# DiWu9/Union-Thesis-SLAM

Hardware: AMD Instinct MI355X
Metric: depth frames/sec (640x480 into 512^3 @ 2 cm dense TSDF; hash alongside) (higher is better)
Workload: dtype f64

## Files before the change

### union-thesis-slam_amd/csrc/tsdf_dense.hip

```cpp
#include <algorithm>
#include <vector>
#include <cstdlib>
#include <cstring>

#include "tsdf_host.h"

using namespace tsdf;

struct tsdf_dense {
    Base b;
    Mesh mesh;
    int nz = 4;
    bool fused = true;
    int gi_per_cu = 0;
};

namespace {

__global__ void k_fill3(float* t, float* w, float* c, size_t n) {
    for (size_t i = (size_t)blockIdx.x * blockDim.x + threadIdx.x; i < n;
         i += (size_t)gridDim.x * blockDim.x) {
        t[i] = 1.0f;
        w[i] = 0.0f;
        c[i] = 0.0f;
// ... 460 lines not shown
        if (e == hipSuccess) e = hipMalloc(&uc, hb);
        if (e == hipSuccess) e = hipMemcpyAsync(ut, halo_tsdf, hb, hipMemcpyHostToDevice, B.stream);
        if (e == hipSuccess) e = hipMemcpyAsync(uc, halo_color, hb, hipMemcpyHostToDevice, B.stream);
        if (e != hipSuccess) r = set_error(TSDF_E_HIP, "halo upload: %s", hipGetErrorString(e));
        ht = ut;
        hc = uc;
    } else if (n_halo > 0) {
        TSDF_HIP(hipDeviceSynchronize());
    }
    if (r == TSDF_OK) r = extract_mesh(B, B.pool, h->mesh, d, ht, hc);
    if (ut) (void)hipFree(ut);
    if (uc) (void)hipFree(uc);
    TSDF_TRY(r);
    *n_verts = h->mesh.n_verts;
    *n_tris = h->mesh.n_tris;
    return TSDF_OK;
}

int tsdf_dense_get_mesh(tsdf_dense_t* h, float* verts, float* normals, uint8_t* colors, int32_t* faces) {
    if (!h) return set_error(TSDF_E_ARG, "null handle");
    TSDF_HIP(hipSetDevice(h->b.device));
    return copy_mesh(h->b, h->mesh, verts, normals, colors, faces);
}

int tsdf_dense_get_mesh_keys(tsdf_dense_t* h, int64_t* keys) {
    if (!h || !keys) return set_error(TSDF_E_ARG, "null pointer");
    TSDF_HIP(hipSetDevice(h->b.device));
    return copy_mesh(h->b, h->mesh, nullptr, nullptr, nullptr, nullptr, keys);
}

int tsdf_dense_get_rows(tsdf_dense_t* h, const int64_t* rows, int64_t n_rows, float* tsdf_, float* weight_,
                        float* color_, int flags) {
    if (!h || n_rows < 0 || (n_rows > 0 && !rows)) return set_error(TSDF_E_ARG, "bad arguments");
    Base& B = h->b;
    TSDF_HIP(hipSetDevice(B.device));
    TSDF_TRY(dense_flush(h));
    if (n_rows == 0) return TSDF_OK;
    for (int64_t i = 0; i < n_rows; ++i)
        if (rows[i] < 0 || rows[i] >= B.vol.dims[0])
            return set_error(TSDF_E_ARG, "local row %lld outside [0, %d)", (long long)rows[i], B.vol.dims[0]);
    const size_t yz = (size_t)B.vol.dims[1] * B.vol.dims[2];
    const size_t bytes = (size_t)n_rows * yz * sizeof(float);
    DevPtrs bufs;
    long long* drows = nullptr;
    TSDF_HIP(hipMalloc(&drows, sizeof(long long) * n_rows));
    bufs.p.push_back(drows);
    TSDF_HIP(hipMemcpyAsync(drows, rows, sizeof(long long) * n_rows, hipMemcpyHostToDevice, B.stream));
    float* out[3] = {tsdf_, weight_, color_};
    float* dev[3] = {B.pool.tsdf, B.pool.weight, B.pool.color};
    const unsigned grid = (unsigned)std::min<size_t>(((size_t)n_rows * yz + 255) / 256, (size_t)B.n_cu * 16);
    for (int k = 0; k < 3; ++k) {
        if (!out[k]) continue;
        float* dst = out[k];
        if (!(flags & TSDF_DEVICE_PTRS)) {
            TSDF_HIP(hipMalloc(&dst, bytes));
            bufs.p.push_back(dst);
        }
        hipLaunchKernelGGL(k_rows<true>, dim3(grid), dim3(256), 0, B.stream, B.vol, (const long long*)drows, 0ll,
                           (long long)n_rows, dev[k], dst);
        TSDF_HIP(hipGetLastError());
        if (!(flags & TSDF_DEVICE_PTRS)) TSDF_HIP(hipMemcpyAsync(out[k], dst, bytes, hipMemcpyDeviceToHost, B.stream));
    }
    TSDF_HIP(hipStreamSynchronize(B.stream));
    return TSDF_OK;
}

int tsdf_dense_set_profiling(tsdf_dense_t* h, int on) {
    if (!h) return set_error(TSDF_E_ARG, "null handle");
    TSDF_HIP(hipSetDevice(h->b.device));
    TSDF_TRY(dense_flush(h));
    return h->b.set_profiling(on);
}

}

#ifdef TSDF_WG_TIMES
extern "C" int tsdf_diag_wg_times(unsigned long long* out) {
    TSDF_HIP(hipDeviceSynchronize());
    TSDF_HIP(hipMemcpyFromSymbol(out, HIP_SYMBOL(g_wg_times), sizeof(unsigned long long) * 4 * kWgTimes));
    static const std::vector<unsigned long long> zero(4 * (size_t)kWgTimes, 0ull);
    TSDF_HIP(hipMemcpyToSymbol(HIP_SYMBOL(g_wg_times), zero.data(), sizeof(unsigned long long) * 4 * kWgTimes));
    return TSDF_OK;
}
#endif

#ifdef TSDF_DIAG
extern "C" int tsdf_diag_counts(unsigned long long* out) {
    TSDF_HIP(hipDeviceSynchronize());
    TSDF_HIP(hipMemcpyFromSymbol(out, HIP_SYMBOL(tsdf::g_ddiag), sizeof(unsigned long long) * 8));
    const unsigned long long zero[8] = {};
    TSDF_HIP(hipMemcpyToSymbol(HIP_SYMBOL(tsdf::g_ddiag), zero, sizeof(zero)));
    return TSDF_OK;
}
#endif
```

### union-thesis-slam_amd/csrc/tsdf_device.h

```cpp
#pragma once
#include <hip/hip_runtime.h>
#include <stdint.h>
#include <type_traits>

namespace tsdf {

constexpr int kBrickEdge = 8;
constexpr int kBrickVox = 512;
constexpr int kWG = 256;
constexpr int kPyrLevels = 6;
constexpr int kStatSpread = 64;
constexpr unsigned long long kEmpty = ~0ull;
constexpr unsigned long long kTomb = ~0ull - 1ull;

enum Stat { ST_VOXELS = 0, ST_VISITED, ST_TOUCHED, ST_ALLOC, ST_PROBE, ST_LOOKUPS, ST_OVERFLOW,
            ST_PROBE_MAX, ST_BAD_ENTRY, ST_UNIQUE, kNStat };

struct Vol {
    int dims[3];
    int off[3];
    int xstride;
    int xodd;
    int sb[3];
    int nb[3];
// ... 97 lines not shown
    long long tombs;
    long long seq;
};

struct Table {
    unsigned long long* keys;
    int* vals;
    unsigned long long* occ;
    int* free_list;
    ListEntry* overflow;
    PoolState* st;
    PoolReport* rb;
    long long capacity;
    long long shard_cap;
    long long max_blocks;
    const int* owned;
    int n_owned;
    int* ins_list;
    long long ins_cap;
    int overflow_cap;
    int int_bits;
};

template <bool POW2 = false>
__host__ __device__ inline long long ref_hash(long long x, long long y, long long z, long long n,
                                              int int_bits) {
    const unsigned long long P1 = 73856093ull, P2 = 19349669ull, P3 = 83492791ull;
    long long h;
    if (int_bits == 32) {
        const int a = (int)(unsigned)((unsigned long long)x * P1);
        const int b = (int)(unsigned)((unsigned long long)y * P2);
        const int c = (int)(unsigned)((unsigned long long)z * P3);
        h = (long long)(a ^ b ^ c);
    } else {
        h = (long long)(((unsigned long long)x * P1) ^ ((unsigned long long)y * P2) ^
                        ((unsigned long long)z * P3));
    }
    if (POW2 || (n & (n - 1)) == 0) return h & (n - 1);
    long long m = h % n;
    return m < 0 ? m + n : m;
}

template <bool POW2 = false>
__host__ __device__ inline int shard_of(long long home, int n_shards, long long cap) {
    if (POW2 || (cap & (cap - 1)) == 0) return (int)((home * n_shards) >> (63 - __builtin_clzll((unsigned long long)cap)));
    return (int)((home * n_shards) / cap);
}

__host__ __device__ inline unsigned long long pack_key(int bx, int by, int bz) {
    return (unsigned long long)bx | ((unsigned long long)by << 21) | ((unsigned long long)bz << 42);
}

__device__ inline int lane_id() { return threadIdx.x & 63; }

__device__ unsigned long long fcmp64_mask(double a, double b, int pred) __asm("llvm.amdgcn.fcmp.i64.f64");
__device__ unsigned long long fcmp32_mask(float a, float b, int pred) __asm("llvm.amdgcn.fcmp.i64.f32");
__device__ unsigned long long icmp32_mask(unsigned a, unsigned b, int pred) __asm("llvm.amdgcn.icmp.i64.i32");
constexpr int kCmpOGT = 2, kCmpOGE = 3, kCmpOLT = 4, kCmpUNE = 14, kCmpNE = 33, kCmpULT = 36, kCmpSGT = 38;
__device__ inline bool lane_in(unsigned long long m) { return __builtin_amdgcn_inverse_ballot_w64(m); }
__device__ inline void sel_in_place(float& x, float y, unsigned long long m) {
    asm("v_cndmask_b32 %0, %0, %1, %2" : "+v"(x) : "v"(y), "s"(m));
}

template <typename T>
__device__ inline T coh_load(T* p) {
    return __hip_atomic_load(p, __ATOMIC_RELAXED, __HIP_MEMORY_SCOPE_AGENT);
}
template <typename T>
__device__ inline void coh_store(T* p, T v) {
    __hip_atomic_store(p, v, __ATOMIC_RELAXED, __HIP_MEMORY_SCOPE_AGENT);
}

__device__ inline double vox_world(float origin, double vs, int g) {
    return (double)(float)((double)origin + vs * (double)g);
}

struct BrickBox {
    double p0[3];
    float ext[3];
    float ctr[3];
    float rad;
};

__device__ inline BrickBox brick_box(const Vol& v, const double* eye, int bx, int by, int bz, int nx = 1,
                                     int ny = 1, int nz = 1) {
    const int bb[3] = {bx, by, bz}, nn[3] = {nx, ny, nz};
    BrickBox r;
#pragma unroll
    for (int a = 0; a < 3; ++a) {
        const int lo = bb[a] * kBrickEdge;
        const int hi = min(lo + nn[a] * kBrickEdge - 1, v.dims[a] - 1);
        const int glo = (a == 0) ? col_gx(v, bb[0]) : lo;
        const int ghi = (a == 0) ? col_gx(v, hi >> 3) + (hi & 7) : hi;
        r.p0[a] = (double)v.origin[a] + v.vs * (double)(glo + v.off[a]);
        r.ext[a] = (float)(v.vs * (double)(ghi - glo));
        r.ctr[a] = (float)(r.p0[a] + 0.5 * v.vs * (double)(ghi - glo) - eye[a]);
    }
    r.rad = 0.5f * sqrtf(r.ext[0] * r.ext[0] + r.ext[1] * r.ext[1] + r.ext[2] * r.ext[2]) + 1e-4f;
    return r;
}

__device__ inline bool cull_brick(const Vol& v, const Frame& fr, const PyrGeo& pg, const BrickBox& bb) {
#pragma unroll
    for (int i = 0; i < 5; ++i) {
        const float* q = fr.planes[i];
        if (q[0] * bb.ctr[0] + q[1] * bb.ctr[1] + q[2] * bb.ctr[2] + q[3] < -bb.rad) return false;
    }
    const double* T = fr.T;
    float c0[3], d[3][3];
#pragma unroll
    for (int r = 0; r < 3; ++r) {
        c0[r] = (float)(T[4 * r + 0] * bb.p0[0] + T[4 * r + 1] * bb.p0[1] + T[4 * r + 2] * bb.p0[2] + T[4 * r + 3]);
#pragma unroll
        for (int a = 0; a < 3; ++a) d[r][a] = (float)T[4 * r + a] * bb.ext[a];
    }
    const float fx = (float)fr.fx, fy = (float)fr.fy, cx = (float)fr.cx, cy = (float)fr.cy;
    float zmin = 3e38f, zmax = -3e38f, umin = 3e38f, umax = -3e38f, vmin = 3e38f, vmax = -3e38f;
#pragma unroll
    for (int c = 0; c < 8; ++c) {
        float q[3];
#pragma unroll
        for (int r = 0; r < 3; ++r)
            q[r] = c0[r] + ((c & 1) ? d[r][0] : 0.0f) + ((c & 2) ? d[r][1] : 0.0f) + ((c & 4) ? d[r][2] : 0.0f);
        zmin = fminf(zmin, q[2]);
        zmax = fmaxf(zmax, q[2]);
        const float iz = __builtin_amdgcn_rcpf(fmaxf(q[2], 1e-6f));
        const float u = fx * q[0] * iz + cx, w = fy * q[1] * iz + cy;
        umin = fminf(umin, u); umax = fmaxf(umax, u);
        vmin = fminf(vmin, w); vmax = fmaxf(vmax, w);
    }
    if (zmax < -1e-4f) return false;
    int u0 = 0, u1 = fr.W - 1, v0 = 0, v1 = fr.H - 1;
    if (zmin > 0.2f) {
        const float fu0 = floorf(umin) - 1.0f, fu1 = ceilf(umax) + 1.0f;
        const float fv0 = floorf(vmin) - 1.0f, fv1 = ceilf(vmax) + 1.0f;
        if (fu1 < 0.0f || fv1 < 0.0f || fu0 > (float)(fr.W - 1) || fv0 > (float)(fr.H - 1)) return false;
        u0 = (int)fmaxf(fu0, 0.0f); u1 = (int)fminf(fu1, (float)(fr.W - 1));
        v0 = (int)fmaxf(fv0, 0.0f); v1 = (int)fminf(fv1, (float)(fr.H - 1));
    }
    int L = 1;
    while (L < kPyrLevels && (((u1 >> L) - (u0 >> L)) > 3 || ((v1 >> L) - (v0 >> L)) > 3)) ++L;
    const float need = zmin - (float)v.trunc - 1e-3f;
    const int tx0 = u0 >> L, tx1 = u1 >> L, ty0 = v0 >> L, ty1 = v1 >> L;
    if (tx1 - tx0 > 3 || ty1 - ty0 > 3) return true;
    const float* lvl = fr.pyr + pg.off[L];
    const int wl = pg.w[L];
    float dmax = 0.0f;
#pragma unroll
    for (int dy = 0; dy < 4; ++dy)
#pragma unroll
        for (int dx = 0; dx < 4; ++dx)
            if (ty0 + dy <= ty1 && tx0 + dx <= tx1) dmax = fmaxf(dmax, lvl[(ty0 + dy) * wl + tx0 + dx]);
    return dmax > 0.0f && dmax >= need;
}

__device__ inline int pool_alloc(const Table& t) {
    const long long c = (long long)atomicAdd((unsigned long long*)&t.st->cursor, 1ull);
    const long long nf = coh_load(&t.st->free_count);
    const long long b = (c < nf) ? (long long)coh_load(&t.free_list[nf - 1 - c])
                                 : coh_load(&t.st->pool_top) + (c - nf);
    return (b < t.max_blocks) ? (int)b : -2;
}

__device__ inline int table_find_or_insert(const Table& t, unsigned long long key, long long home,
                                           bool insert, bool& is_new, long long& slot_out,
                                           long long& probe) {
    const int lane = lane_id();
    is_new = false;
    long long pos = home;
    long long tomb = -1;
    int blk = -1;
    for (long long scanned = 0; scanned < t.capacity + 64;) {
        long long s = pos + lane;
        if (s >= t.capacity) s -= t.capacity;
        if (s >= t.capacity) s %= t.capacity;
        const unsigned long long kk = coh_load(&t.keys[s]);
        const int vv = coh_load(&t.vals[s]);
        const unsigned long long hit = __ballot(kk == key);
        if (hit) {
            const int l = __ffsll((long long)hit) - 1;
            slot_out = __shfl(s, l);
            probe = scanned + l;
            return __shfl(vv, l);
        }
        const unsigned long long emp = __ballot(kk == kEmpty);
        unsigned long long tm = __ballot(kk == kTomb);
        if (emp) tm &= (emp & (~emp + 1)) - 1;
        if (tomb < 0 && tm) tomb = __shfl(s, __ffsll((long long)tm) - 1);
        if (emp) {
            if (!insert) return -1;
            const int le = __ffsll((long long)emp) - 1;
            const long long target = tomb >= 0 ? tomb : __shfl(s, le);
            const unsigned long long expect = tomb >= 0 ? kTomb : kEmpty;
            int ok = 0;
            if (lane == 0) {
                if (blk < 0) blk = pool_alloc(t);
                if (blk >= 0) {
                    const unsigned long long old = atomicCAS(&t.keys[target], expect, key);
                    if (old == expect) {
                        coh_store(&t.vals[target], blk);
                        ok = 1;
                    } else if (old == key) {
                        ok = 2;
                    }
                }
            }
            blk = __shfl(blk, 0);
            ok = __shfl(ok, 0);
            if (blk == -2) return -1;
            if (ok == 1) {
                is_new = true;
                slot_out = target;
                probe = scanned + ((target - pos + t.capacity) % t.capacity);
                return blk;
            }
            if (ok == 2) {
                slot_out = target;
                probe = scanned + ((target - pos + t.capacity) % t.capacity);
                return coh_load(&t.vals[target]);
            }
            scanned += (target - pos + t.capacity) % t.capacity + 1;
            pos = target + 1;
            if (pos >= t.capacity) pos -= t.capacity;
            tomb = -1;
            continue;
        }
        pos += 64;
        if (pos >= t.capacity) pos -= t.capacity;
        scanned += 64;
    }
    return -1;
}


__device__ unsigned short buf_ld_u16(__amdgpu_buffer_rsrc_t r, int vindex, int voffset, int soffset,
                                     int aux) __asm("llvm.amdgcn.struct.ptr.buffer.load.i16");
// ... 651 lines not shown
__device__ inline void append_kept(const Vol& v, ListEntry* list, unsigned int* count, unsigned long long* s_stat,
                                   int* res, unsigned e, unsigned fmask, int ncls, const Table* tab = nullptr,
                                   const Pool* pool = nullptr) {
    const int lane = lane_id();
    const int cls = __popc(fmask);
    const unsigned long long any = __ballot(cls != 0);
    if (!any) return;
    unsigned n_cls = 0, rank = 0;
    for (int c = 1; c <= ncls; ++c) {
        const unsigned long long m = __ballot(cls == c);
        if (lane == c) n_cls = (unsigned)__popcll(m);
        if (cls == c) rank = (unsigned)__popcll(m & ((1ull << lane) - 1ull));
    }
    unsigned base = 0;
    if (lane >= 1 && lane <= ncls && n_cls) base = atomicAdd(&count[lane], n_cls);
    if (lane == 0) atomicAdd(&s_stat[ST_VISITED], (unsigned long long)__popcll(any));
    base = __shfl(base, cls);
    const unsigned nbk = (unsigned)(v.nb[0] * v.nb[1] * v.nb[2]);
    bool fresh = false;
    int blk = kResFree;
    if (cls && base + rank < nbk) {
        list[(size_t)(cls - 1) * nbk + base + rank] = (ListEntry)e | ((ListEntry)fmask << 32);
        if (HASH && res) res[e] = blk = tab ? cull_find_or_insert(v, *tab, e, s_stat, fresh) : kResFree;
    }
    if (HASH && res && pool) {
        for (unsigned long long m = __ballot(fresh); m; m &= m - 1) {
            const int b = __shfl(blk, __ffsll((long long)m) - 1);
            const size_t o = (size_t)b * kBrickVox + (size_t)lane * kBrickEdge;
            const float4 one = make_float4(1.0f, 1.0f, 1.0f, 1.0f), zero = make_float4(0.0f, 0.0f, 0.0f, 0.0f);
            *(float4*)(pool->tsdf + o) = one;
            *(float4*)(pool->tsdf + o + 4) = one;
            *(float4*)(pool->weight + o) = zero;
            *(float4*)(pool->weight + o + 4) = zero;
            *(float4*)(pool->color + o) = zero;
            *(float4*)(pool->color + o + 4) = zero;
            if (lane < kBrickEdge) coh_store(tab->occ + (size_t)b * kBrickEdge + lane, 0ull);
        }
    }
}

constexpr int kCullGMax = 4;
template <bool HASH, bool P2 = false>
__device__ inline void cull_superbrick(const Vol& v, const Batch& bt, const Table& tab, ListEntry* list,
                                       unsigned int* count, unsigned long long* stats, int wgi,
                                       unsigned* s_mask, unsigned long long* s_stat, int* res = nullptr,
                                       int G = 1, const Pool* pool = nullptr) {
    const int tid = threadIdx.x, lane = tid & 63;
    const int wave = __builtin_amdgcn_readfirstlane(tid >> 6), n_waves = (int)(blockDim.x >> 6);
    if (tid < 64 * G) s_mask[tid] = 0u;
    if (tid < kNStat) s_stat[tid] = 0;
    __syncthreads();
    const int nsx = (v.nb[0] + (1 << v.sb[0]) - 1) >> v.sb[0];
    const int nsy = (v.nb[1] + (1 << v.sb[1]) - 1) >> v.sb[1];
    const int nsz = (v.nb[2] + (1 << v.sb[2]) - 1) >> v.sb[2];
    const int n_sb = nsx * nsy * nsz;
    const int ex = 1 << v.sb[0], ey = 1 << v.sb[1], ez = 1 << v.sb[2];
    const int lz = lane & (ez - 1), ly = (lane >> v.sb[2]) & (ey - 1), lx = lane >> (v.sb[1] + v.sb[2]);
    for (int p = wave; p < G * bt.n; p += n_waves) {
        const int g = p / bt.n, f = p - g * bt.n;
        const int si = wgi * G + g;
        if (si >= n_sb) continue;
        const int sx = si / (nsy * nsz), sr = si - sx * (nsy * nsz), sy = sr / nsz, sz = sr - sy * nsz;
        const int bx = sx * ex + lx, by = sy * ey + ly, bz = sz * ez + lz;
        const Frame& fr = bt.f[f];
        bool test = bx < v.nb[0] && by < v.nb[1] && bz < v.nb[2];
        if (HASH && v.n_shards > 1 && test) {
            const long long home = ref_hash<P2>(bx, by, bz, tab.shard_cap, tab.int_bits);
            test = shard_of<P2>(home, v.n_shards, tab.shard_cap) == v.shard;
        }
        if (test && cull_brick(v, fr, bt.pg, brick_box(v, fr.eye, bx, by, bz))) atomicOr(&s_mask[g * 64 + lane], 1u << f);
    }
    __syncthreads();
    const int si = wgi * G + wave;
    if (wave < G && si < n_sb) {
        const int sx = si / (nsy * nsz), sr = si - sx * (nsy * nsz), sy = sr / nsz, sz = sr - sy * nsz;
        const int bx = sx * ex + lx, by = sy * ey + ly, bz = sz * ez + lz;
        append_kept<HASH>(v, list, count, s_stat, res, (unsigned)(((long long)bx * v.nb[1] + by) * v.nb[2] + bz),
                          s_mask[wave * 64 + lane], bt.n, P2 ? &tab : nullptr, pool);
    }
    __syncthreads();
    flush_stats(s_stat, stats);
}

#ifndef TSDF_CULL_WAVE_PRIO
#define TSDF_CULL_WAVE_PRIO 3
#endif
#ifndef TSDF_PAIR_SKEW
#define TSDF_PAIR_SKEW 20
#endif
#ifndef TSDF_TAIL_PRIO
#define TSDF_TAIL_PRIO 0
#endif
__device__ inline void cull_units(const Vol& v, const Batch& bt, ListEntry* list, unsigned int* count,
                                  unsigned long long* s_stat) {
    const int lane = lane_id();
    const int nsx = (v.nb[0] + (1 << v.sb[0]) - 1) >> v.sb[0];
    const int nsy = (v.nb[1] + (1 << v.sb[1]) - 1) >> v.sb[1];
    const int nsz = (v.nb[2] + (1 << v.sb[2]) - 1) >> v.sb[2];
    const unsigned n_sb = (unsigned)(nsx * nsy * nsz);
    const int n = __builtin_amdgcn_readfirstlane(bt.n);
    bool prio = false;
    for (;;) {
        unsigned u = 0;
        if (lane == 0) u = atomicAdd(&count[kCursorWord], 1u);
        u = __builtin_amdgcn_readfirstlane(u);
        if (u >= n_sb) break;
        if (TSDF_CULL_WAVE_PRIO && !prio) {
            __builtin_amdgcn_s_setprio(TSDF_CULL_WAVE_PRIO);
            prio = true;
        }
        const int si = (int)u;
        const int lz = lane & ((1 << v.sb[2]) - 1), ly = (lane >> v.sb[2]) & ((1 << v.sb[1]) - 1);
        const int lx = lane >> (v.sb[1] + v.sb[2]);
        const int sx = si / (nsy * nsz), sr = si - sx * (nsy * nsz), sy = sr / nsz, sz = sr - sy * nsz;
        const int bx = (sx << v.sb[0]) + lx, by = (sy << v.sb[1]) + ly, bz = (sz << v.sb[2]) + lz;
        const bool test = bx < v.nb[0] && by < v.nb[1] && bz < v.nb[2];
        unsigned fmask = 0;
#pragma unroll 2
        for (int f = 0; f < n; ++f) {
            const Frame& fr = bt.f[f];
            if (test && cull_brick(v, fr, bt.pg, brick_box(v, fr.eye, bx, by, bz))) fmask |= 1u << f;
        }
        append_kept<false>(v, list, count, s_stat, nullptr, (unsigned)(((long long)bx * v.nb[1] + by) * v.nb[2] + bz),
                           fmask, n);
    }
    if (TSDF_CULL_WAVE_PRIO && prio) __builtin_amdgcn_s_setprio(0);
}

template <bool HASH>
__device__ inline void cull_owned(const Vol& v, const Batch& bt, const Table& tab, ListEntry* list,
                                  unsigned int* count, unsigned long long* stats, int wgi, unsigned* s_mask,
                                  unsigned long long* s_stat, int* res, const Pool* pool = nullptr) {
    const int tid = threadIdx.x, lane = tid & 63;
    const int wave = __builtin_amdgcn_readfirstlane(tid >> 6), n_waves = (int)(blockDim.x >> 6);
    if (tid < 64) s_mask[tid] = 0u;
    if (tid < kNStat) s_stat[tid] = 0;
    __syncthreads();
    const int i = wgi * 64 + lane;
    const bool have = i < tab.n_owned;
    const int e = have ? tab.owned[i] : 0;
    const int nb12 = v.nb[1] * v.nb[2];
    const int bx = e / nb12, r = e - bx * nb12, by = r / v.nb[2], bz = r - by * v.nb[2];
    for (int f = wave; f < bt.n; f += n_waves) {
        const Frame& fr = bt.f[f];
        if (have && cull_brick(v, fr, bt.pg, brick_box(v, fr.eye, bx, by, bz))) atomicOr(&s_mask[lane], 1u << f);
    }
    __syncthreads();
    if (wave == 0) append_kept<HASH>(v, list, count, s_stat, res, (unsigned)e, have ? s_mask[lane] : 0u, bt.n, &tab, pool);
    __syncthreads();
    flush_stats(s_stat, stats);
}

template <bool HASH>
__global__ __launch_bounds__(kCullWG) void k_cull(Vol v, Batch bt, Table tab, ListEntry* list,
                                                  unsigned int* count, unsigned long long* stats) {
    __shared__ unsigned s_mask[64];
    __shared__ unsigned long long s_stat[kNStat];
    if (HASH && tab.owned) cull_owned<HASH>(v, bt, tab, list, count, stats, blockIdx.x, s_mask, s_stat, nullptr);
    else cull_superbrick<HASH>(v, bt, tab, list, count, stats, blockIdx.x, s_mask, s_stat);
}

#ifndef TSDF_PRIO
#define TSDF_PRIO 1
#endif
#ifndef TSDF_PRIO_HASH
#define TSDF_PRIO_HASH 1
#endif
#ifndef TSDF_PRIO_MIN
#define TSDF_PRIO_MIN 64
#endif
#ifndef TSDF_PRIO_MIN_HASH
#define TSDF_PRIO_MIN_HASH 16
#endif
template <typename T>
__device__ inline const __attribute__((address_space(4))) T* opaque(const __attribute__((address_space(4))) T* p) {
    asm volatile("" : "+s"(p));
    return p;
}

typedef const __attribute__((address_space(4))) Vol* VolP;
__device__ inline const Vol& item_vol(const Vol& v) { return *(const Vol*)opaque((VolP)&v); }

template <bool HASH, int DK, int CK, bool OW1, int NZ, bool CU>
__device__ inline void integrate_items(const Vol& v, const Batch& bt, const Pool& pool, const Table& tab,
                                       const ListEntry* list, unsigned int* count, int n_list, int wave,
                                       int n_waves, unsigned long long* s_stat, const double* s_rcp,
                                       unsigned* s_next, int wg, int n_wg, int* res, unsigned& nupd,
                                       unsigned& nuniq, int skew);
template <bool HASH, int DK, int CK, bool OW1, int NZ, bool CU = false>
__device__ inline void integrate_list(const Vol& v, const Batch& bt, const Pool& pool, const Table& tab,
                                      const ListEntry* list, unsigned int* count, int n_list, int wave,
                                      int n_waves, unsigned long long* s_stat, const double* s_rcp,
                                      unsigned* s_next = nullptr, int wg = 0, int n_wg = 1, int* res = nullptr,
                                      int skew = 0) {
    wave = __builtin_amdgcn_readfirstlane(wave);
    unsigned nupd = 0, nuniq = 0;
    integrate_items<HASH, DK, CK, OW1, NZ, CU>(v, bt, pool, tab, list, count, n_list, wave, n_waves, s_stat, s_rcp,
                                           s_next, wg, n_wg, res, nupd, nuniq, skew);
    if (lane_id() == 0 && nupd) {
        atomicAdd(&s_stat[ST_VOXELS], (unsigned long long)nupd);
        atomicAdd(&s_stat[ST_UNIQUE], (unsigned long long)nuniq);
    }
}

template <bool HASH, int DK, int CK, bool OW1, int NZ, bool CU>
__device__ inline void integrate_items(const Vol& v, const Batch& bt, const Pool& pool, const Table& tab,
                                       const ListEntry* list, unsigned int* count, int n_list, int wave,
// ... 278 lines not shown
    sa[r][c] = m1;
    __syncthreads();
    pyr_level<0>(bt.pg, pyr, 2, sa, sb, 16);
    __syncthreads();
    pyr_level<0>(bt.pg, pyr, 3, sb, sa, 8);
    __syncthreads();
    pyr_level<0>(bt.pg, pyr, 4, sa, sb, 4);
    __syncthreads();
    pyr_level<0>(bt.pg, pyr, 5, sb, sa, 2);
    __syncthreads();
    pyr_level<0>(bt.pg, pyr, 6, sa, sb, 1);
}

#ifndef TSDF_FUSED_WG
#define TSDF_FUSED_WG 768
#endif
#ifndef TSDF_FUSED_HASH_WG
#define TSDF_FUSED_HASH_WG 768
#endif
constexpr int kFusedWG = TSDF_FUSED_WG, kFusedHashWG = TSDF_FUSED_HASH_WG;
static_assert(kFusedWG >= kCullWG && kFusedHashWG >= kCullWG && kFusedWG % 64 == 0 && kFusedHashWG % 64 == 0,
              "a cull workgroup is one wave per frame of the batch");
struct Stage {
    const ListEntry* list_i;
    unsigned int* count_i;
    ListEntry* list_c;
    unsigned int* count_c;
    unsigned int* count_p;
    int gi, gc;
    int cw;
    int cg;
    int ptx, pty;
    long long seq;
    int* res_i;
    int* res_c;
    unsigned* done;
};

#ifdef TSDF_WG_TIMES
constexpr int kWgTimes = 16384;
__device__ unsigned long long g_wg_times[4][kWgTimes];
__device__ inline unsigned long long wg_place() {
    unsigned hw, xcc;
    asm volatile("s_getreg_b32 %0, hwreg(HW_REG_HW_ID)" : "=s"(hw));
    asm volatile("s_getreg_b32 %0, hwreg(HW_REG_XCC_ID)" : "=s"(xcc));
    return ((unsigned long long)xcc << 32) | hw;
}
#endif
struct FusedArgs {
    Vol v;
    Batch bi, bc, bp;
    Pool pool;
    unsigned long long* stats;
    Stage sg;
};
typedef const __attribute__((address_space(4))) FusedArgs* FusedArgsP;

template <bool OW1, int NZ, int DK = 0, bool CU = false>
__global__ __launch_bounds__(kFusedWG) __attribute__((amdgpu_waves_per_eu(TSDF_DENSE_WAVES))) void k_fused(FusedArgs a) {
    const FusedArgsP A = (FusedArgsP)__builtin_amdgcn_kernarg_segment_ptr();
    const Vol& v = *(const Vol*)opaque(&A->v);
    const Pool& pool = *(const Pool*)opaque(&A->pool);
    const Batch &bi = a.bi, &bc = a.bc, &bp = a.bp;
    unsigned long long* const stats = a.stats;
    const Stage& sg = a.sg;
    __shared__ double s_buf[kRcpTab];
    __shared__ unsigned long long s_stat[kNStat];
    __shared__ unsigned s_next;
    const int tid = threadIdx.x, b = blockIdx.x;
    const Table no_table{};
#ifdef TSDF_WG_TIMES
    const bool rec = sg.gi > 0 && (sg.gc > 0 || sg.cw > 0) &&(int)gridDim.x > sg.gi + sg.gc && b < kWgTimes;
    if (tid == 0 && rec) g_wg_times[0][b] = __builtin_amdgcn_s_memrealtime();
#endif
    if (b < sg.gi) {
        if (tid < kNStat) s_stat[tid] = 0;
        if (tid == 0) s_next = 0;
        if (OW1)
            for (int i = tid; i < kRcpTab / 2; i += kFusedWG) ((double2*)s_buf)[i] = ((const double2*)v.rcp)[i];
        __syncthreads();
        constexpr int wpg = kFusedWG / 64;
        const int cw = __builtin_amdgcn_readfirstlane(sg.cw);
        if (cw > 0 && __builtin_amdgcn_readfirstlane(tid >> 6) >= wpg - cw)
            cull_units(item_vol(v), bc, sg.list_c, sg.count_c, s_stat);
        integrate_list<false, DK, 0, OW1, NZ, CU>(v, bi, pool, no_table, sg.list_i, sg.count_i, 0,
                                             b * wpg + (tid >> 6), sg.gi * wpg, s_stat,
                                             OW1 ? s_buf : nullptr, &s_next, b, sg.gi, nullptr,
                                             cw > 0 ? TSDF_PAIR_SKEW : 0);
        if (cw > 0) cull_units(item_vol(v), bc, sg.list_c, sg.count_c, s_stat);
        __syncthreads();
        flush_stats(s_stat, stats);
    } else if (b < sg.gi + sg.gc) {
        if (TSDF_TAIL_PRIO) __builtin_amdgcn_s_setprio(TSDF_TAIL_PRIO);
        cull_superbrick<false>(v, bc, no_table, sg.list_c, sg.count_c, stats, b - sg.gi, (unsigned*)s_buf,
                               s_stat, nullptr, sg.cg);
    } else {
        if (TSDF_TAIL_PRIO) __builtin_amdgcn_s_setprio(TSDF_TAIL_PRIO);
        const int t = b - sg.gi - sg.gc, per = sg.ptx * sg.pty;
        const int f = t / per, r = t - f * per;
        float(*sa)[33] = (float(*)[33])s_buf;
        prep_vec_tile<DK>(bp, sg.count_p, r % sg.ptx, r / sg.ptx, f, sa, sa + 32);
    }
#ifdef TSDF_WG_TIMES
    __syncthreads();
    if (tid == 0 && rec) {
        g_wg_times[1][b] = __builtin_amdgcn_s_memrealtime();
        g_wg_times[3][b] = wg_place();
        g_wg_times[2][b] = ((unsigned long long)(b < sg.gi ? 0 : b < sg.gi + sg.gc ? 1 : 2) << 32) |
                           (b < sg.gi ? s_next : 0u);
    }
#endif
}

__device__ inline void commit_pool(PoolState* st, long long max_blocks, PoolReport* rb = nullptr,
                                   long long seq = -1, const unsigned* count = nullptr) {
    const long long used = coh_load(&st->cursor);
    const long long nf = coh_load(&st->free_count);
    const long long cons = used < nf ? used : nf;
    long long top = coh_load(&st->pool_top) + (used - cons);
    top = top < max_blocks ? top : max_blocks;
    coh_store(&st->free_count, nf - cons);
    coh_store(&st->pool_top, top);
    coh_store(&st->cursor, 0ll);
    if (rb && seq >= 0) {
        PoolReport* r = rb + (seq % kReports);
        __hip_atomic_store(&r->pool_top, top, __ATOMIC_RELAXED, __HIP_MEMORY_SCOPE_SYSTEM);
        __hip_atomic_store(&r->free_count, nf - cons, __ATOMIC_RELAXED, __HIP_MEMORY_SCOPE_SYSTEM);
        __hip_atomic_store(&r->n_overflow, coh_load(&st->n_overflow), __ATOMIC_RELAXED, __HIP_MEMORY_SCOPE_SYSTEM);
        __hip_atomic_store(&r->tombs, coh_load(&st->tombs), __ATOMIC_RELAXED, __HIP_MEMORY_SCOPE_SYSTEM);
        long long listed = 0;
        if (count)
            for (int c = 1; c <= kMaxBatch; ++c) listed += coh_load(&((unsigned*)count)[c]);
        __hip_atomic_store(&r->listed, listed, __ATOMIC_RELAXED, __HIP_MEMORY_SCOPE_SYSTEM);
        __hip_atomic_store(&r->seq, seq + 1, __ATOMIC_RELEASE, __HIP_MEMORY_SCOPE_SYSTEM);
    }
}

#ifndef TSDF_FUSED_HASH_WAVES
#define TSDF_FUSED_HASH_WAVES 6
#endif
struct FusedHashArgs {
    Vol v;
    Batch bi, bc, bp;
    Pool pool;
    Table tab;
    unsigned long long* stats;
    Stage sg;
};

template <int DK = 0, bool CU = false>
__global__ __launch_bounds__(kFusedHashWG) __attribute__((amdgpu_waves_per_eu(TSDF_FUSED_HASH_WAVES))) void k_fused_hash(
        FusedHashArgs a) {
    typedef const __attribute__((address_space(4))) FusedHashArgs* ArgsP;
    const ArgsP A = (ArgsP)__builtin_amdgcn_kernarg_segment_ptr();
    const Table& tab = *(const Table*)opaque(&A->tab);
    const Vol& v = *(const Vol*)opaque(&A->v);
    const Pool& pool = *(const Pool*)opaque(&A->pool);
    const Batch &bi = a.bi, &bc = a.bc, &bp = a.bp;
    unsigned long long* const stats = a.stats;
    const Stage& sg = a.sg;
    __shared__ double s_buf[kRcpTab];
    __shared__ unsigned long long s_stat[kNStat];
    __shared__ int s_last;
    __shared__ unsigned s_next;
    const int tid = threadIdx.x, b = blockIdx.x;
#ifdef TSDF_WG_TIMES
    const bool rec = sg.gi > 0 && sg.gc > 0 && (int)gridDim.x > sg.gi + sg.gc && b < kWgTimes;
    if (tid == 0 && rec) g_wg_times[0][b] = __builtin_amdgcn_s_memrealtime();
#endif
    if (b < sg.gi) {
        if (tid < kNStat) s_stat[tid] = 0;
        if (tid == 0) s_next = 0;
// ... 44 lines not shown
```

Baseline: 26320.

## Restructure cull_units into lane-distributed frame loads with two-pass sphere and projection culling

```diff
diff --git a/union-thesis-slam_amd/csrc/tsdf_dense.hip b/union-thesis-slam_amd/csrc/tsdf_dense.hip
--- a/union-thesis-slam_amd/csrc/tsdf_dense.hip
+++ b/union-thesis-slam_amd/csrc/tsdf_dense.hip
@@ -566,6 +566,13 @@
     TSDF_HIP(hipMemcpyToSymbol(HIP_SYMBOL(g_wg_times), zero.data(), sizeof(unsigned long long) * 4 * kWgTimes));
     return TSDF_OK;
 }
+extern "C" int tsdf_diag_unit_times(unsigned long long* out) {
+    TSDF_HIP(hipDeviceSynchronize());
+    TSDF_HIP(hipMemcpyFromSymbol(out, HIP_SYMBOL(g_unit_times), sizeof(unsigned long long) * 4 * kUnitTimes));
+    static const std::vector<unsigned long long> zero(4 * (size_t)kUnitTimes, 0ull);
+    TSDF_HIP(hipMemcpyToSymbol(HIP_SYMBOL(g_unit_times), zero.data(), sizeof(unsigned long long) * 4 * kUnitTimes));
+    return TSDF_OK;
+}
 #endif
 
 #ifdef TSDF_DIAG
diff --git a/union-thesis-slam_amd/csrc/tsdf_device.h b/union-thesis-slam_amd/csrc/tsdf_device.h
--- a/union-thesis-slam_amd/csrc/tsdf_device.h
+++ b/union-thesis-slam_amd/csrc/tsdf_device.h
@@ -203,10 +203,16 @@
     float rad;
 };
 
-__device__ inline BrickBox brick_box(const Vol& v, const double* eye, int bx, int by, int bz, int nx = 1,
-                                     int ny = 1, int nz = 1) {
+struct BrickGeom {
+    double p0[3];
+    double mid[3];
+    float ext[3];
+    float rad;
+};
+
+__device__ inline BrickGeom brick_geom(const Vol& v, int bx, int by, int bz, int nx = 1, int ny = 1, int nz = 1) {
     const int bb[3] = {bx, by, bz}, nn[3] = {nx, ny, nz};
-    BrickBox r;
+    BrickGeom r;
 #pragma unroll
     for (int a = 0; a < 3; ++a) {
         const int lo = bb[a] * kBrickEdge;
@@ -215,27 +221,67 @@
         const int ghi = (a == 0) ? col_gx(v, hi >> 3) + (hi & 7) : hi;
         r.p0[a] = (double)v.origin[a] + v.vs * (double)(glo + v.off[a]);
         r.ext[a] = (float)(v.vs * (double)(ghi - glo));
-        r.ctr[a] = (float)(r.p0[a] + 0.5 * v.vs * (double)(ghi - glo) - eye[a]);
+        r.mid[a] = r.p0[a] + 0.5 * v.vs * (double)(ghi - glo);
     }
     r.rad = 0.5f * sqrtf(r.ext[0] * r.ext[0] + r.ext[1] * r.ext[1] + r.ext[2] * r.ext[2]) + 1e-4f;
     return r;
 }
 
-__device__ inline bool cull_brick(const Vol& v, const Frame& fr, const PyrGeo& pg, const BrickBox& bb) {
+__device__ inline BrickBox brick_box(const Vol& v, const double* eye, int bx, int by, int bz, int nx = 1,
+                                     int ny = 1, int nz = 1) {
+    const BrickGeom g = brick_geom(v, bx, by, bz, nx, ny, nz);
+    BrickBox r;
+#pragma unroll
+    for (int a = 0; a < 3; ++a) {
+        r.p0[a] = g.p0[a];
+        r.ext[a] = g.ext[a];
+        r.ctr[a] = (float)(g.mid[a] - eye[a]);
+    }
+    r.rad = g.rad;
+    return r;
+}
+
+__device__ inline bool cull_sphere(const float (&planes)[5][4], const float* ctr, float rad) {
 #pragma unroll
     for (int i = 0; i < 5; ++i) {
-        const float* q = fr.planes[i];
-        if (q[0] * bb.ctr[0] + q[1] * bb.ctr[1] + q[2] * bb.ctr[2] + q[3] < -bb.rad) return false;
-    }
+        const float* q = planes[i];
+        if (q[0] * ctr[0] + q[1] * ctr[1] + q[2] * ctr[2] + q[3] < -rad) return false;
+    }
+    return true;
+}
+
+struct CullFrame {
+    double T[12];
+    float fx, fy, cx, cy;
+    int W, H;
+    const float* pyr;
+};
+__device__ inline CullFrame cull_frame(const Frame& fr) {
+    CullFrame c;
+#pragma unroll
+    for (int i = 0; i < 12; ++i) c.T[i] = fr.T[i];
+    c.fx = (float)fr.fx; c.fy = (float)fr.fy; c.cx = (float)fr.cx; c.cy = (float)fr.cy;
+    c.W = fr.W; c.H = fr.H;
+    c.pyr = fr.pyr;
+    return c;
+}
+
+constexpr int kCullDrop = 0, kCullKeep = 1, kCullProbe = 2;
+struct DepthProbe {
+    int tx0, tx1, ty0, ty1, off, wl;
+    float need;
+};
+__device__ inline int cull_project(const Vol& v, const CullFrame& fr, const PyrGeo& pg, const double* p0,
+                                   const float* ext, DepthProbe& pr) {
     const double* T = fr.T;
     float c0[3], d[3][3];
 #pragma unroll
     for (int r = 0; r < 3; ++r) {
-        c0[r] = (float)(T[4 * r + 0] * bb.p0[0] + T[4 * r + 1] * bb.p0[1] + T[4 * r + 2] * bb.p0[2] + T[4 * r + 3]);
-#pragma unroll
-        for (int a = 0; a < 3; ++a) d[r][a] = (float)T[4 * r + a] * bb.ext[a];
-    }
-    const float fx = (float)fr.fx, fy = (float)fr.fy, cx = (float)fr.cx, cy = (float)fr.cy;
+        c0[r] = (float)(T[4 * r + 0] * p0[0] + T[4 * r + 1] * p0[1] + T[4 * r + 2] * p0[2] + T[4 * r + 3]);
+#pragma unroll
+        for (int a = 0; a < 3; ++a) d[r][a] = (float)T[4 * r + a] * ext[a];
+    }
+    const float fx = fr.fx, fy = fr.fy, cx = fr.cx, cy = fr.cy;
     float zmin = 3e38f, zmax = -3e38f, umin = 3e38f, umax = -3e38f, vmin = 3e38f, vmax = -3e38f;
 #pragma unroll
     for (int c = 0; c < 8; ++c) {
@@ -250,29 +296,56 @@
         umin = fminf(umin, u); umax = fmaxf(umax, u);
         vmin = fminf(vmin, w); vmax = fmaxf(vmax, w);
     }
-    if (zmax < -1e-4f) return false;
+    bool drop = zmax < -1e-4f;
     int u0 = 0, u1 = fr.W - 1, v0 = 0, v1 = fr.H - 1;
     if (zmin > 0.2f) {
         const float fu0 = floorf(umin) - 1.0f, fu1 = ceilf(umax) + 1.0f;
         const float fv0 = floorf(vmin) - 1.0f, fv1 = ceilf(vmax) + 1.0f;
-        if (fu1 < 0.0f || fv1 < 0.0f || fu0 > (float)(fr.W - 1) || fv0 > (float)(fr.H - 1)) return false;
-        u0 = (int)fmaxf(fu0, 0.0f); u1 = (int)fminf(fu1, (float)(fr.W - 1));
-        v0 = (int)fmaxf(fv0, 0.0f); v1 = (int)fminf(fv1, (float)(fr.H - 1));
+        drop |= fu1 < 0.0f || fv1 < 0.0f || fu0 > (float)(fr.W - 1) || fv0 > (float)(fr.H - 1);
+        u0 = (int)fminf(fmaxf(fu0, 0.0f), (float)(fr.W - 1)); u1 = (int)fmaxf(fminf(fu1, (float)(fr.W - 1)), 0.0f);
+        v0 = (int)fminf(fmaxf(fv0, 0.0f), (float)(fr.H - 1)); v1 = (int)fmaxf(fminf(fv1, (float)(fr.H - 1)), 0.0f);
     }
     int L = 1;
     while (L < kPyrLevels && (((u1 >> L) - (u0 >> L)) > 3 || ((v1 >> L) - (v0 >> L)) > 3)) ++L;
-    const float need = zmin - (float)v.trunc - 1e-3f;
-    const int tx0 = u0 >> L, tx1 = u1 >> L, ty0 = v0 >> L, ty1 = v1 >> L;
-    if (tx1 - tx0 > 3 || ty1 - ty0 > 3) return true;
-    const float* lvl = fr.pyr + pg.off[L];
-    const int wl = pg.w[L];
+    pr.need = zmin - (float)v.trunc - 1e-3f;
+    pr.tx0 = u0 >> L; pr.tx1 = u1 >> L; pr.ty0 = v0 >> L; pr.ty1 = v1 >> L;
+    pr.off = pg.off[1];
+    pr.wl = pg.w[1];
+#pragma unroll
+    for (int l = 2; l <= kPyrLevels; ++l) {
+        pr.off = L >= l ? pg.off[l] : pr.off;
+        pr.wl = L >= l ? pg.w[l] : pr.wl;
+    }
+    if (drop) return kCullDrop;
+    return (pr.tx1 - pr.tx0 > 3 || pr.ty1 - pr.ty0 > 3) ? kCullKeep : kCullProbe;
+}
+
+template <bool CLAMP>
+__device__ inline void probe_load(const float* pyr, const DepthProbe& pr, float (&t)[16]) {
+    const float* lvl = pyr + pr.off;
+#pragma unroll
+    for (int dy = 0; dy < 4; ++dy)
+#pragma unroll
+        for (int dx = 0; dx < 4; ++dx) {
+            if (CLAMP) t[dy * 4 + dx] = lvl[(unsigned)(min(pr.ty0 + dy, pr.ty1) * pr.wl + min(pr.tx0 + dx, pr.tx1))];
+            else t[dy * 4 + dx] = (pr.ty0 + dy <= pr.ty1 && pr.tx0 + dx <= pr.tx1) ? lvl[(pr.ty0 + dy) * pr.wl + pr.tx0 + dx] : 0.0f;
+        }
+}
+__device__ inline bool probe_keep(float need, const float (&t)[16]) {
     float dmax = 0.0f;
 #pragma unroll
-    for (int dy = 0; dy < 4; ++dy)
-#pragma unroll
-        for (int dx = 0; dx < 4; ++dx)
-            if (ty0 + dy <= ty1 && tx0 + dx <= tx1) dmax = fmaxf(dmax, lvl[(ty0 + dy) * wl + tx0 + dx]);
+    for (int i = 0; i < 16; ++i) dmax = fmaxf(dmax, t[i]);
     return dmax > 0.0f && dmax >= need;
+}
+
+__device__ inline bool cull_brick(const Vol& v, const Frame& fr, const PyrGeo& pg, const BrickBox& bb) {
+    if (!cull_sphere(fr.planes, bb.ctr, bb.rad)) return false;
+    DepthProbe pr;
+    const int res = cull_project(v, cull_frame(fr), pg, bb.p0, bb.ext, pr);
+    if (res != kCullProbe) return res == kCullKeep;
+    float t[16];
+    probe_load<false>(fr.pyr, pr, t);
+    return probe_keep(pr.need, t);
 }
 
 __device__ inline int pool_alloc(const Table& t) {
@@ -1090,6 +1163,16 @@
     flush_stats(s_stat, stats);
 }
 
+__device__ inline float readlane_f32(float x, int l) {
+    return __uint_as_float(__builtin_amdgcn_readlane(__float_as_uint(x), l));
+}
+#ifdef TSDF_WG_TIMES
+constexpr int kUnitTimes = 8192;
+__device__ unsigned long long g_unit_times[4][kUnitTimes];
+#endif
+#ifndef TSDF_CULL_PAIR
+#define TSDF_CULL_PAIR 0
+#endif
 #ifndef TSDF_CULL_WAVE_PRIO
 #define TSDF_CULL_WAVE_PRIO 3
 #endif
@@ -1099,14 +1182,15 @@
 #ifndef TSDF_TAIL_PRIO
 #define TSDF_TAIL_PRIO 0
 #endif
-__device__ inline void cull_units(const Vol& v, const Batch& bt, ListEntry* list, unsigned int* count,
+typedef const __attribute__((address_space(4))) Batch* BatchP;
+__device__ __forceinline__ void cull_units(const Vol& v, BatchP bt, ListEntry* list, unsigned int* count,
                                   unsigned long long* s_stat) {
     const int lane = lane_id();
     const int nsx = (v.nb[0] + (1 << v.sb[0]) - 1) >> v.sb[0];
     const int nsy = (v.nb[1] + (1 << v.sb[1]) - 1) >> v.sb[1];
     const int nsz = (v.nb[2] + (1 << v.sb[2]) - 1) >> v.sb[2];
     const unsigned n_sb = (unsigned)(nsx * nsy * nsz);
-    const int n = __builtin_amdgcn_readfirstlane(bt.n);
+    const int n = __builtin_amdgcn_readfirstlane(bt->n);
     bool prio = false;
     for (;;) {
         unsigned u = 0;
@@ -1123,14 +1207,117 @@
         const int sx = si / (nsy * nsz), sr = si - sx * (nsy * nsz), sy = sr / nsz, sz = sr - sy * nsz;
         const int bx = (sx << v.sb[0]) + lx, by = (sy << v.sb[1]) + ly, bz = (sz << v.sb[2]) + lz;
         const bool test = bx < v.nb[0] && by < v.nb[1] && bz < v.nb[2];
+#ifdef TSDF_WG_TIMES
+        const unsigned long long t_start = __builtin_amdgcn_s_memrealtime();
+#endif
+        int li = lane & (kMaxBatch - 1);
+        asm volatile("" : "+v"(li));
+        const Batch& bu = *(const Batch*)bt;
+        const Frame& fl = bu.f[li];
+        static_assert(offsetof(Frame, eye) == offsetof(Frame, planes) + sizeof(float) * 20, "planes, then eye");
+        const bool hi = lane >= 32;
+        unsigned wl[13];
+        {
+            const unsigned* blk = (const unsigned*)&fl.planes[0][0] + (hi ? 13 : 0);
+#pragma unroll
+            for (int i = 0; i < 13; ++i) wl[i] = blk[i];
+        }
+        BrickGeom g = brick_geom(v, bx, by, bz);
+        unsigned cand = 0, wmask = 0;
+        for (int f = 0; f < n; ++f) {
+            unsigned w[26];
+#pragma unroll
+            for (int i = 0; i < 13; ++i) {
+                w[i] = __builtin_amdgcn_readlane(wl[i], f);
+                w[13 + i] = __builtin_amdgcn_readlane(wl[i], f + 32);
+            }
+            float q[5][4], ctr[3];
+#pragma unroll
+            for (int i = 0; i < 20; ++i) q[i >> 2][i & 3] = __uint_as_float(w[i]);
+#pragma unroll
+            for (int a = 0; a < 3; ++a)
+                ctr[a] = (float)(g.mid[a] - __longlong_as_double((long long)(w[20 + 2 * a] | ((unsigned long long)w[21 + 2 * a] << 32))));
+            const bool c = test && cull_sphere(q, ctr, g.rad);
+            cand |= c ? 1u << f : 0u;
+            wmask |= __ballot(c) ? 1u << f : 0u;
+        }
+#ifdef TSDF_WG_TIMES
+        const unsigned long long t_pass1 = __builtin_amdgcn_s_memrealtime();
+#endif
         unsigned fmask = 0;
-#pragma unroll 2
-        for (int f = 0; f < n; ++f) {
-            const Frame& fr = bt.f[f];
-            if (test && cull_brick(v, fr, bt.pg, brick_box(v, fr.eye, bx, by, bz))) fmask |= 1u << f;
-        }
-        append_kept<false>(v, list, count, s_stat, nullptr, (unsigned)(((long long)bx * v.nb[1] + by) * v.nb[2] + bz),
-                           fmask, n);
+        if (wmask) {
+            int cx = bx;
+            asm volatile("" : "+v"(cx));
+            g = brick_geom(v, cx, by, bz);
+            double Tl[6];
+            {
+                const double* Tp = fl.T + (hi ? 6 : 0);
+#pragma unroll
+                for (int i = 0; i < 6; ++i) Tl[i] = Tp[i];
+            }
+            const double kd[4] = {fl.fx, fl.fy, fl.cx, fl.cy};
+            const unsigned long long pp = (unsigned long long)fl.pyr;
+            const unsigned hw[4] = {(unsigned)fl.W, (unsigned)fl.H, (unsigned)pp, (unsigned)(pp >> 32)};
+            unsigned xl[4];
+#pragma unroll
+            for (int i = 0; i < 4; ++i) xl[i] = hi ? hw[i] : __float_as_uint((float)kd[i]);
+            auto project = [&](int f, DepthProbe& pr, const float*& pyr) __attribute__((always_inline)) {
+                CullFrame fc;
+#pragma unroll
+                for (int i = 0; i < 6; ++i) {
+                    fc.T[i] = readlane_f64(Tl[i], f);
+                    fc.T[6 + i] = readlane_f64(Tl[i], f + 32);
+                }
+                fc.fx = __uint_as_float(__builtin_amdgcn_readlane(xl[0], f));
+                fc.fy = __uint_as_float(__builtin_amdgcn_readlane(xl[1], f));
+                fc.cx = __uint_as_float(__builtin_amdgcn_readlane(xl[2], f));
+                fc.cy = __uint_as_float(__builtin_amdgcn_readlane(xl[3], f));
+                fc.W = (int)__builtin_amdgcn_readlane(xl[0], f + 32);
+                fc.H = (int)__builtin_amdgcn_readlane(xl[1], f + 32);
+                const unsigned plo = (unsigned)__builtin_amdgcn_readlane(xl[2], f + 32);
+                const unsigned phi = (unsigned)__builtin_amdgcn_readlane(xl[3], f + 32);
+                pyr = fc.pyr = (const float*)((unsigned long long)plo | ((unsigned long long)phi << 32));
+                return cull_project(v, fc, bu.pg, g.p0, g.ext, pr);
+            };
+            auto finish = [&](int f, int res, float need, const float (&t)[16]) __attribute__((always_inline)) {
+                const bool keep = res == kCullKeep || (res == kCullProbe && probe_keep(need, t));
+                fmask |= (keep && ((cand >> f) & 1u)) ? 1u << f : 0u;
+            };
+            for (unsigned m = wmask; m;) {
+                DepthProbe pa, pb;
+                const float *pyra, *pyrb;
+                float ta[16], tb[16];
+                const int fa = __builtin_ctz(m);
+                m &= m - 1;
+                const int ra = project(fa, pa, pyra);
+                const bool two = TSDF_CULL_PAIR && m;
+                const int fb = two ? __builtin_ctz(m) : 0;
+                int rb = kCullDrop;
+                if (two) {
+                    m &= m - 1;
+                    rb = project(fb, pb, pyrb);
+                }
+                probe_load<true>(pyra, pa, ta);
+                if (two) {
+                    probe_load<true>(pyrb, pb, tb);
+                    finish(fa, ra, pa.need, ta);
+                    finish(fb, rb, pb.need, tb);
+                } else {
+                    finish(fa, ra, pa.need, ta);
+                }
+            }
+        }
+        const unsigned e = (unsigned)(((long long)bx * v.nb[1] + by) * v.nb[2] + bz);
+        append_kept<false>(v, list, count, s_stat, nullptr, e, fmask, n);
+#ifdef TSDF_WG_TIMES
+        const unsigned long long kept = __ballot(fmask != 0);
+        if (lane == 0 && u < (unsigned)kUnitTimes) {
+            g_unit_times[0][u] = t_start;
+            g_unit_times[1][u] = t_pass1;
+            g_unit_times[2][u] = __builtin_amdgcn_s_memrealtime();
+            g_unit_times[3][u] = (unsigned long long)__popc(wmask) | ((unsigned long long)__popcll(kept) << 32);
+        }
+#endif
     }
     if (TSDF_CULL_WAVE_PRIO && prio) __builtin_amdgcn_s_setprio(0);
 }
@@ -1575,12 +1762,12 @@
         constexpr int wpg = kFusedWG / 64;
         const int cw = __builtin_amdgcn_readfirstlane(sg.cw);
         if (cw > 0 && __builtin_amdgcn_readfirstlane(tid >> 6) >= wpg - cw)
-            cull_units(item_vol(v), bc, sg.list_c, sg.count_c, s_stat);
+            cull_units(item_vol(v), &A->bc, sg.list_c, sg.count_c, s_stat);
         integrate_list<false, DK, 0, OW1, NZ, CU>(v, bi, pool, no_table, sg.list_i, sg.count_i, 0,
                                              b * wpg + (tid >> 6), sg.gi * wpg, s_stat,
                                              OW1 ? s_buf : nullptr, &s_next, b, sg.gi, nullptr,
                                              cw > 0 ? TSDF_PAIR_SKEW : 0);
-        if (cw > 0) cull_units(item_vol(v), bc, sg.list_c, sg.count_c, s_stat);
+        if (cw > 0) cull_units(item_vol(v), &A->bc, sg.list_c, sg.count_c, s_stat);
         __syncthreads();
         flush_stats(s_stat, stats);
     } else if (b < sg.gi + sg.gc) {
```

After: 26380, median of 5. Within noise of the previous version (+0.2%).
